# huster-wgm/SRCGAN

Hardware: AMD Instinct MI355X
Metric: paired SR-CycleGAN train images/sec at x4 256->1024 (higher is better)
Workload: dtype bf16; 1 GPU; Sat2Aerx4 paired G+D step (BASELINE configs[1]): 23-block RRDB generator + 3-layer PatchGAN, 3x256x256->3x1024x1024, batch 16/GPU; per_gpu_batch=16, global_batch=16, parallelism=dp1, gradient_exchange=none (1 rank)

## Files before the change

include/srcgan_amd.h:

```cpp
#ifndef SRCGAN_AMD_H
#define SRCGAN_AMD_H

#include <stddef.h>
#include <stdint.h>

#ifdef __cplusplus
extern "C" {
#endif

#define SRCGAN_F32 0
#define SRCGAN_BF16 1
#define SRCGAN_F16 2

int srcgan_version(void);
const char* srcgan_last_error(void);
int srcgan_dtype_size(int dtype);

int srcgan_nchw_f32_to_nhwc(const float* src, void* dst, int B, int C, int H, int W,
                            int cs, int dtype, void* stream);
int srcgan_nhwc_to_nchw_f32(const void* src, float* dst, int B, int C, int H, int W,
                            int cs, int coff, int dtype, void* stream);

size_t srcgan_packed_weight_bytes(int rows, int kdim, int ntaps, int dtype);
int srcgan_pack_weight(const float* w, void* wp, int rows, int kdim, int tys, int txs,
// ... 19 lines not shown
    long x_plane, y_plane, r1_plane, r2_plane, mz_plane;
    int rev_batch;
    void* sign_out; const void* sign_in;
    int npar; long wpar_stride;
} srcgan_conv_desc;
int srcgan_conv_igemm(const srcgan_conv_desc* d, void* stream);

typedef struct srcgan_wgrad_desc {
    const void* dy; const void* x; float* slab; float* grad;
    float* bias_grad;
    int dtype;
    int kh, kw, stride;
    int B, H, W, Cin, x_cs, x_coff;
    int OH, OW, Cout, dy_cs, dy_coff;
    int pad_y, pad_x;
    int nsplit;
    long sr, sk, sty, stx, off;
    float alpha;
    int accumulate;
} srcgan_wgrad_desc;
size_t srcgan_conv_wgrad_slab_bytes(int Cout, int Cin, int kh, int kw, int nsplit);
int srcgan_conv_wgrad_nsplit(int B, int OH, int OW, int Cout, int Cin, int stride);
int srcgan_conv_wgrad(const srcgan_wgrad_desc* d, void* stream);

typedef struct srcgan_wgrad_seg { int g0, g1; float* grad; float* bias; int Cin; float alpha; } srcgan_wgrad_seg;
typedef struct srcgan_wgrad_dense_desc {
    const void* dy; const void* x; float* slab;
    int dtype;
    int B, H, W;
    int G, dy_cs, dy_coff;
    int C, x_cs, x_coff;
    int nseg;
    srcgan_wgrad_seg seg[8];
    int accumulate;
    long dy_plane, x_plane;
} srcgan_wgrad_dense_desc;
size_t srcgan_wgrad_dense_slab_bytes(int G, int C, int dtype, int B, int H, int W);
int srcgan_wgrad_dense(const srcgan_wgrad_dense_desc* d, void* stream);

int srcgan_col_reduce_blocks(long npix);
int srcgan_col_reduce(int mode, const void* a, int a_cs, int a_coff, const void* z, int z_cs, int z_coff,
                      const float* m, const float* rstd, long npix, int C, float scale,
                      float* out0, float* out1, float* scratch, int dtype, void* stream);

int srcgan_bn_finalize(const float* mean, const float* var, float* rstd, float* running_mean,
                       float* running_var, int64_t* num_batches_tracked, int C, long count,
// ... 353 lines not shown
```

srcgan_amd/_native.py:

```python
from __future__ import annotations

import ctypes as C
import os
from typing import Optional, Sequence

import torch

_HERE = os.path.dirname(os.path.abspath(__file__))
LIB_PATH = os.environ.get("SRCGAN_AMD_LIB") or os.path.join(_HERE, "lib", "libsrcgan_amd.so")

F32, BF16, F16 = 0, 1, 2
_DTYPES = {"fp32": F32, "f32": F32, "float32": F32, torch.float32: F32,
           "bf16": BF16, "bfloat16": BF16, torch.bfloat16: BF16,
           "fp16": F16, "f16": F16, "float16": F16, "half": F16, torch.float16: F16, F32: F32, BF16: BF16, F16: F16}
_default_dtype = _DTYPES[os.environ.get("SRCGAN_AMD_DTYPE", "fp32")]


def dtype_id(d) -> int:
    if d is None:
        return _default_dtype
    try:
        return _DTYPES[d]
    except KeyError:
        raise ValueError(f"unsupported compute dtype {d!r} (use 'fp32', 'bf16' or 'fp16')") from None
# ... 27 lines not shown

class WgradDesc(C.Structure):
    _fields_ = [("dy", C.c_void_p), ("x", C.c_void_p), ("slab", C.c_void_p), ("grad", C.c_void_p), ("bias_grad", C.c_void_p),
                ("dtype", C.c_int), ("kh", C.c_int), ("kw", C.c_int), ("stride", C.c_int),
                ("B", C.c_int), ("H", C.c_int), ("W", C.c_int), ("Cin", C.c_int), ("x_cs", C.c_int), ("x_coff", C.c_int),
                ("OH", C.c_int), ("OW", C.c_int), ("Cout", C.c_int), ("dy_cs", C.c_int), ("dy_coff", C.c_int),
                ("pad_y", C.c_int), ("pad_x", C.c_int), ("nsplit", C.c_int),
                ("sr", C.c_long), ("sk", C.c_long), ("sty", C.c_long), ("stx", C.c_long), ("off", C.c_long),
                ("alpha", C.c_float), ("accumulate", C.c_int)]


class WgradSeg(C.Structure):
    _fields_ = [("g0", C.c_int), ("g1", C.c_int), ("grad", C.c_void_p), ("bias", C.c_void_p), ("Cin", C.c_int), ("alpha", C.c_float)]


class WgradDenseDesc(C.Structure):
    _fields_ = [("dy", C.c_void_p), ("x", C.c_void_p), ("slab", C.c_void_p), ("dtype", C.c_int),
                ("B", C.c_int), ("H", C.c_int), ("W", C.c_int),
                ("G", C.c_int), ("dy_cs", C.c_int), ("dy_coff", C.c_int),
                ("C", C.c_int), ("x_cs", C.c_int), ("x_coff", C.c_int),
                ("nseg", C.c_int), ("seg", WgradSeg * 8), ("accumulate", C.c_int), ("dy_plane", C.c_long), ("x_plane", C.c_long)]


class RddbCfg(C.Structure):
    _fields_ = [("in_ch", C.c_int), ("out_ch", C.c_int), ("up", C.c_int), ("nf", C.c_int), ("nb", C.c_int), ("gc", C.c_int),
                ("B", C.c_int), ("H", C.c_int), ("W", C.c_int), ("dtype", C.c_int), ("down", C.c_int), ("legacy", C.c_int)]


class NetOpts(C.Structure):
    _fields_ = [("wpack", C.c_void_p), ("pack", C.c_int), ("rrdb_lo", C.c_int), ("rrdb_hi", C.c_int), ("guard", C.c_void_p)]


class ResDeconvCfg(C.Structure):
    _fields_ = [("in_ch", C.c_int), ("out_ch", C.c_int), ("B", C.c_int), ("H", C.c_int), ("W", C.c_int), ("dtype", C.c_int),
                ("layers", C.c_int * 4), ("norm", C.c_int)]


class SrNetCfg(C.Structure):
    _fields_ = [(n, C.c_int) for n in ("kind", "in_ch", "out_ch", "up", "base", "B", "H", "W", "dtype", "nres")]


class SrDenseCfg(C.Structure):
    _fields_ = [(n, C.c_int) for n in ("kind", "in_ch", "out_ch", "B", "H", "W", "dtype", "growth", "num_blocks", "num_layers", "up")]


class RcanCfg(C.Structure):
# ... 20 lines not shown
class VggLossCfg(C.Structure):
    _fields_ = [(n, C.c_int) for n in ("kind", "B", "H", "W", "dtype")]


class NLayerDCfg(C.Structure):
    _fields_ = [("in_ch", C.c_int), ("ndf", C.c_int), ("n_layers", C.c_int),
                ("B", C.c_int), ("H", C.c_int), ("W", C.c_int), ("dtype", C.c_int), ("training", C.c_int), ("norm", C.c_int)]


_P, _I, _L, _F, _S = C.c_void_p, C.c_int, C.c_long, C.c_float, C.c_size_t
SIGNATURES = {
    "srcgan_version": (_I, []),
    "srcgan_last_error": (C.c_char_p, []),
    "srcgan_dtype_size": (_I, [_I]),
    "srcgan_nchw_f32_to_nhwc": (_I, [_P, _P, _I, _I, _I, _I, _I, _I, _P]),
    "srcgan_nhwc_to_nchw_f32": (_I, [_P, _P, _I, _I, _I, _I, _I, _I, _I, _P]),
    "srcgan_packed_weight_bytes": (_S, [_I, _I, _I, _I]),
    "srcgan_pack_weight": (_I, [_P, _P, _I, _I, _I, _I, _L, _L, _L, _L, _L, _I, _P]),
    "srcgan_pack_weight_part": (_I, [_P, _P, _I, _I, _I, _I, _L, _L, _L, _L, _L, _I, _I, _F, _I, _P]),
    "srcgan_conv_igemm": (_I, [C.POINTER(ConvDesc), _P]),
    "srcgan_conv_wgrad_slab_bytes": (_S, [_I, _I, _I, _I, _I]),
    "srcgan_conv_wgrad_nsplit": (_I, [_I, _I, _I, _I, _I, _I]),
    "srcgan_conv_wgrad": (_I, [C.POINTER(WgradDesc), _P]),
    "srcgan_wgrad_dense_slab_bytes": (_S, [_I, _I, _I, _I, _I, _I]),
    "srcgan_wgrad_dense": (_I, [C.POINTER(WgradDenseDesc), _P]),
    "srcgan_col_reduce_blocks": (_I, [_L]),
    "srcgan_col_reduce": (_I, [_I, _P, _I, _I, _P, _I, _I, _P, _P, _L, _I, _F, _P, _P, _P, _I, _P]),
    "srcgan_bn_finalize": (_I, [_P, _P, _P, _P, _P, _P, _I, _L, _F, _F, _P]),
    "srcgan_bn_eval_rstd": (_I, [_P, _P, _I, _F, _P]),
    "srcgan_bn_apply_lrelu": (_I, [_P, _P, _P, _P, _P, _P, _L, _I, _I, _F, _I, _P]),
    "srcgan_bn_bwd_apply": (_I, [_P, _P, _P, _P, _P, _P, _P, _P, _L, _I, _I, _I, _P]),
    "srcgan_add_inplace": (_I, [_P, _I, _I, _P, _I, _I, _P, _I, _I, _F, _L, _I, _I, _P]),
    "srcgan_add_inplace_planes": (_I, [_P, _I, _I, _L, _P, _I, _I, _L, _P, _I, _I, _L, _F, _L, _I, _I, _P]),
    "srcgan_gn_scratch_floats": (_S, [_I, _I]),
    "srcgan_gn_forward": (_I, [_P, _I, _P, _I, _P, _I, _P, _P, _P, _I, _L, _I, _I, _F, _I, _F, _I, _P, _P]),
    "srcgan_gn_backward": (_I, [_P, _I, _P, _I, _P, _I, _P, _P, _P, _I, _P, _I, _I, _P, _P, _I, _F, _I, _L, _I, _I, _I, _P, _P]),
    "srcgan_ca_scratch_floats": (_S, [_I, _L, _I]),
    "srcgan_ca_forward": (_I, [_P, _I, _P, _I, _P, _I, _P, _P, _P, _P, _P, _I, _L, _I, _I, _I, _P, _P]),
    "srcgan_ca_backward": (_I, [_P, _I, _P, _I, _P, _P, _P, _P, _I, _P, _I, _I, _P, _P, _P, _P, _I, _L, _I, _I, _I, _P, _P]),
    "srcgan_s2d_shift": (_I, [_P, _I, _P, _I, _I, _I, _I, _I, _I, _I, _I, _I, _I, _P]),
    "srcgan_d2s_shift": (_I, [_P, _I, _P, _I, _I, _I, _I, _I, _I, _I, _I, _I, _I, _I, _P]),
    "srcgan_prelu_forward": (_I, [_P, _I, _P, _P, _P, _I, _F, _P, _I, _I, _I, _I, _I, _I, _I, _I, _I, _I, _P]),
    "srcgan_prelu_scratch_floats": (_S, [_I, _I, _I, _I, _I]),
    "srcgan_prelu_backward": (_I, [_P, _I, _P, _I, _P, _P, _P, _I, _P, _I, _F, _I, _P, _P, _I, _I, _I, _I, _I, _I, _I, _I, _I, _P, _P]),
    "srcgan_upsample2_nhwc": (_I, [_P, _I, _I, _L, _P, _I, _I, _I, _I, _I, _I, _P]),
    "srcgan_sum2x2_nhwc": (_I, [_P, _I, _P, _I, _P, _I, _F, _I, _I, _I, _I, _I, _P]),
# ... 191 lines not shown
```

srcgan_amd/build.py:

```python
import glob
import os
import subprocess
import sys
from concurrent.futures import ThreadPoolExecutor

HERE = os.path.dirname(os.path.abspath(__file__))
CSRC = os.path.join(HERE, "csrc")
LIBDIR = os.path.join(HERE, "lib")
LIB = os.path.join(LIBDIR, "libsrcgan_amd.so")
SOURCES = ["conv_entry.hip", "conv_igemm.hip", "conv_par4.hip", "deconv_k3s2.hip", "conv3x3_dma.hip", "conv_wgrad.hip", "wgrad_dense.hip", "elementwise.hip", "class_losses.hip", "groupnorm.hip", "chan_attn.hip", "back_proj.hip", "metrics.hip", "shift_select.hip", "scene_score.hip", "colour.hip", "tiles.hip", "vgg_loss.hip", "nets.hip", "oplist.hip"]
FLAGS = ["--offload-arch=gfx950", "-O3", "-std=c++17", "-fPIC", "-Wall", "-Wno-unused-function"]


def _hipcc():
    for c in (os.environ.get("HIPCC"), "/opt/rocm/bin/hipcc", "hipcc"):
        if c and (os.path.isabs(c) and os.path.exists(c) or not os.path.isabs(c)):
            return c
    raise RuntimeError("hipcc not found")


def _stale(target, deps):
    if not os.path.exists(target):
        return True
    t = os.path.getmtime(target)
    return any(os.path.getmtime(d) > t for d in deps)


def build(force=False, verbose=True):
    os.makedirs(LIBDIR, exist_ok=True)
    hipcc = _hipcc()
    headers = glob.glob(os.path.join(CSRC, "*.h")) + [os.path.join(HERE, "..", "include", "srcgan_amd.h")]
    objs, jobs = [], []
    for s in SOURCES:
# ... 23 lines not shown
```

srcgan_amd/csrc/common.h:

```cpp
#pragma once
#include <hip/hip_runtime.h>
#include <stdint.h>
#include <stdio.h>
#include <stdarg.h>
#include <string.h>
#include "../../include/srcgan_amd.h"

typedef __attribute__((ext_vector_type(8))) __bf16 bf16x8;
typedef __attribute__((ext_vector_type(8))) _Float16 f16x8;
typedef __attribute__((ext_vector_type(4))) _Float16 f16x4;
typedef __attribute__((ext_vector_type(4))) __bf16 bf16x4;
typedef __attribute__((ext_vector_type(4))) float f32x4;
typedef __attribute__((ext_vector_type(16))) float f32x16;
typedef __attribute__((ext_vector_type(4))) short s16x4;
typedef __attribute__((ext_vector_type(4))) unsigned int u32x4;
typedef __attribute__((ext_vector_type(2))) unsigned int u32x2;

template <typename T> struct DT;
template <> struct DT<float>  { static constexpr int id = SRCGAN_F32;  static constexpr int EPP = 4; static constexpr int KCE = 16; };
template <> struct DT<__bf16> { static constexpr int id = SRCGAN_BF16; static constexpr int EPP = 8; static constexpr int KCE = 32; };
template <> struct DT<_Float16> { static constexpr int id = SRCGAN_F16; static constexpr int EPP = 8; static constexpr int KCE = 32; };
static inline bool sg_is16(int dtype) { return dtype == SRCGAN_BF16 || dtype == SRCGAN_F16; }
static inline bool sg_dtype_ok(int dtype) { return dtype == SRCGAN_F32 || sg_is16(dtype); }

// ... 79 lines not shown
#endif
#endif

int sg_prof_start(const char* cls, double flops, double bytes, hipStream_t st);
void sg_prof_stop(int token, hipStream_t st);

struct SgPackJob {
    const float* w; size_t wp_off;
    int rows, kdim, tys, txs;
    long sr, sk, sty, stx, off;
    int k_off, k_total; float scale;
    int cot, nchunk; long total, blk0;
};
void sg_pack_job_finish(SgPackJob& j, int dtype, long& blk_cursor);
int sg_pack_multi_launch(const SgPackJob* jobs_dev, int njobs, long nblocks, void* wp_base, int dtype, hipStream_t st, const unsigned long long* guard = nullptr);
int sg_fold_tail_pack(const float* w_deconv, const float* w_conv, void* wp, int tar, int dtype, hipStream_t st);
void sg_minmax_frames(const float* x, int planes, int frames, long n, int nblk, float* partial, float* range, hipStream_t st);
int sg_vgg_combine(const float* sums, const float* weights, int n, float* out, hipStream_t st);
struct SgFrames { int Cin, F, f0, k; };
int sg_frames_pack(const float* src5d, void* dst, int cs, int Bt, SgFrames fr, int H, int W, int dtype, hipStream_t st);
int sg_frames_grad_store(const void* src, int cs, float* dst5d, int Bt, SgFrames fr, int H, int W, const float* gout, float gscale, int dtype, hipStream_t st);
int sg_meanshift(const void* x, void* y, const float* w, const float* bias, int transpose, long npix, int dtype, hipStream_t st);
int sg_proj_repack(const float* src, float* dst, int form, int rows, int kdim, int k, int s, int back, hipStream_t st);
int sg_fill_zero_guarded(void* p, size_t bytes, const unsigned long long* guard, hipStream_t st);
```

srcgan_amd/csrc/conv_wgrad.hip:

```cpp
#include "launch.h"
#include <type_traits>

struct WgradP {
    const void* dy; const void* x; float* slab;
    int B, H, W, Cin, xCs, xcoff;
    int OH, OW, Cout, dyCs, dycoff;
    int pad_y, pad_x;
    int nsplit, tiles_x, tiles_y, ntiles, citiles, ctiles, want_bias;
};

typedef __attribute__((address_space(3))) s16x4 lds_s16x4;

__device__ __forceinline__ bf16x8 tr_frag(const char* p0, const char* p1) {
    s16x4 lo = __builtin_amdgcn_ds_read_tr16_b64_v4i16((lds_s16x4*)(p0));
    s16x4 hi = __builtin_amdgcn_ds_read_tr16_b64_v4i16((lds_s16x4*)(p1));
    typedef __attribute__((ext_vector_type(8))) short s16x8;
    s16x8 v = {lo[0], lo[1], lo[2], lo[3], hi[0], hi[1], hi[2], hi[3]};
    return __builtin_bit_cast(bf16x8, v);
}

template <typename T, int KH, int KW, int S, int MT, int TH, int NCW, bool BIASW>
__global__ __launch_bounds__((NCW + (BIASW ? 1 : 0)) * 64) void conv_wgrad_k(const WgradP p) {
    using D = DT<T>;
    constexpr int NW = NCW + (BIASW ? 1 : 0);
// ... 323 lines not shown
        s = (a0 + a1) + (a2 + a3);
    }
    red[sl][el] = s;
    __syncthreads();
    if (sl != 0 || e >= per_split) return;
    s = (red[0][el] + red[1][el]) + (red[2][el] + red[3][el]);
    long q = e;
    const int ci_l = (int)(q % 32); q /= 32;
    const int co_l = (int)(q % p.COT); q /= p.COT;
    const int tap = (int)(q % (p.ntap + 1)); q /= (p.ntap + 1);
    const int cit = (int)(q % p.citiles);
    const int ct = (int)(q / p.citiles);
    const int co = ct * p.COT + co_l, ci = cit * 32 + ci_l;
    if (co >= p.Cout) return;
    const float v = s * p.alpha;
    if (tap == p.ntap) {
        if (p.bias_grad && cit == 0 && ci_l == 0) p.bias_grad[co] = p.accumulate ? p.bias_grad[co] + v : v;
        return;
    }
    if (ci >= p.Cin) return;
    const int ky = tap / p.kw, kx = tap % p.kw;
    float* g = p.grad + p.off + co * p.sr + ci * p.sk + ky * p.sty + kx * p.stx;
    *g = p.accumulate ? (*g + v) : v;
}

static inline int wg_cot(int Cout) { return Cout <= 32 ? 32 : 64; }

extern "C" size_t srcgan_conv_wgrad_slab_bytes(int Cout, int Cin, int kh, int kw, int nsplit) {
    const int cot = wg_cot(Cout);
    return (size_t)nsplit * cdiv(Cout, cot) * cdiv(Cin, 32) * (kh * kw + 1) * cot * 32 * sizeof(float);
}

extern "C" int srcgan_conv_wgrad_nsplit(int B, int OH, int OW, int Cout, int Cin, int stride) {
    const int th = stride == 2 ? 4 : 8;
    const long ntiles = (long)B * cdiv(OH, th) * cdiv(OW, 32);
    const long pairs = (long)cdiv(Cout, wg_cot(Cout)) * cdiv(Cin, 32);
    long want = cdivl(1024, pairs);
    if (want > ntiles) want = ntiles;
    if (want > 256) want = 256;
    if (want < 1) want = 1;
    return (int)want;
}

template <typename T, int KH, int KW, int S, int MT, int TH, int NCW, bool BIASW>
static int launch_wgrad(WgradP p, hipStream_t st) {
    constexpr int NW = NCW + (BIASW ? 1 : 0);
// ... 69 lines not shown
    int rc;
    const bool c3 = d->kh == 3 && d->kw == 3 && d->Cout <= 3 && d->OH == d->H && d->OW == d->W;
    const bool c1 = d->kh == 4 && d->kw == 4 && d->Cout == 1 && d->OH == d->H - 1 && d->OW == d->W - 1;
    if (sg_is16(d->dtype) && (c3 || c1) && d->stride == 1 && d->pad_y == 1 && d->pad_x == 1 && !d->bias_grad && d->Cin % 32 == 0) {
        p.tiles_x = cdiv(p.W, 32); p.tiles_y = cdiv(p.H, 8); p.ntiles = p.B * p.tiles_x * p.tiles_y;
        p.nsplit = d->nsplit;
        if (p.nsplit > p.ntiles) p.nsplit = p.ntiles;
        const dim3 grid((unsigned)(p.citiles * ((p.nsplit + 7) / 8) * 8), 1, 1);
        const double px = (double)p.B * p.OH * p.OW;
        rc = sg_dtype_dispatch16(d->dtype, [&](auto t) {
            using T = decltype(t);
            char cls[96];
            snprintf(cls, sizeof(cls), "conv_wgrad<%s,%s>", sg_dtype_tag<T>(), c3 ? "3x3,s1,c3" : "4x4,s1,c1");
            const int tok = sg_prof_start(cls, 2.0 * px * d->kh * d->kw * d->Cin * d->Cout, ((double)p.B * p.H * p.W * d->Cin + px * d->Cout) * 2, st);
            if (c3) hipLaunchKernelGGL((wgrad_c3_k<T, 3, 3>), grid, dim3(256), 0, st, p);
            else hipLaunchKernelGGL((wgrad_c3_k<T, 4, 1>), grid, dim3(256), 0, st, p);
            sg_prof_stop(tok, st);
            SG_LAUNCH_CHECK();
            return 0;
        });
    } else if (cot == 32) rc = sg_dtype_dispatch(d->dtype, [&](auto t) { return dispatch_wgrad<decltype(t), 1>(p, d->kh, d->kw, d->stride, st); });
    else rc = sg_dtype_dispatch(d->dtype, [&](auto t) { return dispatch_wgrad<decltype(t), 2>(p, d->kh, d->kw, d->stride, st); });
    if (rc) return rc;
    WredP q;
    q.slab = d->slab; q.grad = d->grad; q.bias_grad = d->bias_grad; q.nsplit = p.nsplit; q.ctiles = p.ctiles; q.citiles = p.citiles;
    q.ntap = d->kh * d->kw; q.kw = d->kw; q.COT = cot; q.Cout = d->Cout; q.Cin = d->Cin;
    q.sr = d->sr; q.sk = d->sk; q.sty = d->sty; q.stx = d->stx; q.off = d->off;
    q.alpha = d->alpha; q.accumulate = d->accumulate;
    const long per_split = (long)p.ctiles * p.citiles * (q.ntap + 1) * cot * 32;
    hipLaunchKernelGGL(wgrad_reduce_k, dim3((unsigned)cdivl(per_split, 64)), dim3(256), 0, st, q);
    SG_LAUNCH_CHECK();
    return 0;
}
```

srcgan_amd/csrc/nets.hip:

```cpp
#include "net_common.h"
#include <map>
#include <mutex>
#include <string>

int sg_zigzag_next() {
    static const bool zig = sg_env("SRCGAN_NO_ZIGZAG") == nullptr;
    static int flip = 0;
    const int rev = flip;
    flip ^= 1;
    return zig ? rev : 0;
}

namespace {
struct PackCache { std::vector<SgPackJob> host; SgPackJob* dev = nullptr; SgPackJob* pinned = nullptr; size_t cap = 0; hipEvent_t staged = nullptr; };
std::map<std::string, PackCache> g_pack_cache;
std::mutex g_pack_mutex;
}

int sg_pack_list_run(const std::vector<SgPackJob>& jobs, long nblk, void* wp_base, int dtype, const char* tag, const void* key_ptr, void* st,
                     const unsigned long long* guard) {
    if (jobs.empty()) return 0;
    int dev = 0;
    SG_HIP(hipGetDevice(&dev));
    char key[112];
// ... 198 lines not shown
    }
    if (P.nrr) N.home = b.take((size_t)((nf + P.kce - 1) / P.kce) * P.plane_bytes);
    if (P.family != RDDB_LEGACY) N.T = b.take(B * P.Ht * P.Wt * nf * e);
    if (P.x2_tail) {
        N.U[0] = b.take(B * P.Ht * P.Wt * nf * e);
        size_t pp[2];
        for (int k = 0; k < 2; ++k) pp[k] = b.take(B * P.HO * P.WO * nf * e);
        for (int k = 0; k < P.ntail; ++k) N.tail[k] = pp[k & 1];
    } else if (P.family == RDDB_SRDN) {
        N.U[0] = N.T;
    } else {
        size_t pp[2] = {0, 0};
        for (int k = 0; k < 2 && k <= P.nst; ++k) {
            const int top = ((P.nst - k) & ~1) + k;
            pp[k] = b.take(B * (P.Ht << top) * (P.Wt << top) * nf * e);
        }
        for (int s = 0; s <= P.nst; ++s) N.U[s] = pp[s & 1];
    }
    N.out = b.take(B * P.HO * P.WO * P.out_cs * e);
    N.wpk = b.off;
    N.total = N.wpk + P.wpack_bytes;
}

struct RddbBwdPlan {
    size_t dout, dU[6], Pg[3], szP, dfea_dn[5], dxin, slab, colscr, total;
};
static void rddb_bwd_plan(const srcgan_rddbnet_cfg* c, const RddbPlan& P, RddbBwdPlan& Q) {
    const size_t e = P.esz, B = c->B;
    Bump b;
    Q.dout = b.take(B * P.HO * P.WO * P.out_cs * e);
    for (int s = 0; s <= P.nup; ++s) Q.dU[s] = b.take(B * (P.Ht << s) * (P.Wt << s) * c->nf * e);
    if (P.x2_tail) { Q.dU[1] = b.take(B * P.HO * P.WO * c->nf * e); Q.dU[2] = b.take(B * P.HO * P.WO * c->nf * e); }
    Q.szP = align_up((size_t)P.nplane * P.plane_bytes, 256);
    for (int i = 0; i < 3; ++i) Q.Pg[i] = b.take(Q.szP);
    for (int s = 0; s <= P.ndn; ++s) Q.dfea_dn[s] = b.take(B * (c->H >> s) * (c->W >> s) * c->nf * e);
    Q.dxin = b.take(B * c->H * c->W * P.in_cs * e);
    size_t slab = 0;
    auto mx = [&](size_t v) { if (v > slab) slab = v; };
    mx(wgrad_slab(c->B, c->H, c->W, c->nf, P.in_cs, 3, 3, 1));
    for (int k = 0; k < 5; ++k) mx(wgrad_slab(c->B, P.Ht, P.Wt, k < 4 ? c->gc : c->nf, c->nf + k * c->gc, 3, 3, 1));
    mx(wgrad_slab(c->B, P.Ht, P.Wt, c->nf, c->nf, 3, 3, 1));
    for (int s = 0; s < P.nup; ++s) mx(wgrad_slab(c->B, P.Ht << s, P.Wt << s, c->nf, c->nf, 2, 2, 2));
    for (int k = 0; k < P.ntail; ++k) if (P.tail[k].conv) mx(wgrad_slab(c->B, P.tail[k].hout, P.tail[k].wout, c->nf, c->nf, 3, 3, 1));
    for (int s = 0; s < P.ndn; ++s) mx(wgrad_slab(c->B, c->H >> (s + 1), c->W >> (s + 1), c->nf, c->nf, 3, 3, 2));
    mx(wgrad_slab(c->B, P.HO, P.WO, c->out_ch, c->nf, 3, 3, 1));
    mx(srcgan_wgrad_dense_slab_bytes(P.C, P.C, c->dtype, c->B, P.Ht, P.Wt));
    Q.slab = b.take(slab);
    const long maxpix = (long)B * (P.HO > c->H ? P.HO : c->H) * (P.WO > c->W ? P.WO : c->W);
    Q.colscr = b.take((size_t)2 * srcgan_col_reduce_blocks(maxpix) * P.C * sizeof(float));
    Q.total = b.off + 256;
}

}

extern "C" int srcgan_rddbnet_num_params(const srcgan_rddbnet_cfg* c) { RddbPlan P; if (rddb_plan(c, P)) return -1; return P.nparams; }
extern "C" int srcgan_rddbnet_num_rrdb(const srcgan_rddbnet_cfg* c) { RddbPlan P; if (rddb_plan(c, P)) return -1; return P.nrr; }
extern "C" size_t srcgan_rddbnet_wpack_bytes(const srcgan_rddbnet_cfg* c) { RddbPlan P; if (rddb_plan(c, P)) return 0; return P.wpack_bytes; }
extern "C" size_t srcgan_rddbnet_ws_bytes(const srcgan_rddbnet_cfg* c) {
    RddbPlan P; if (rddb_plan(c, P)) return 0;
    RddbNames N; rddb_train_names(c, P, N); return N.total;
}
extern "C" size_t srcgan_rddbnet_infer_ws_bytes(const srcgan_rddbnet_cfg* c) {
    RddbPlan P; if (rddb_plan(c, P)) return 0;
    RddbNames N; rddb_infer_names(c, P, N); return N.total;
}
// ... 207 lines not shown
        }
    }
    for (int s = 0; s < P.ndn; ++s) P.dn_dgrad().pack(packs, params[P.p_dn0 + 2 * s], wp, P.w_dn_d[s]);
    if (pack_dx) packs.add(params[P.p_first_w], wp + P.w_first_d, c->in_ch, nf, 3, 3, lay_dgrad_s1(c->in_ch, 3, 3));
    return packs.run((std::string(P.tag) + (pack_dx ? "_bwd_dx" : "_bwd")).c_str(), params[0], st, pack_guard(opt));
}

int RddbBwd::output_plain() const {
    TRef Ul = T_(N.U[P.nup], nf);
    if (G(P.p_last_w))
        SG_TRY(wgrad_call(dt, dout(), P.HO, P.WO, c->out_ch, Ul, B, P.HO, P.WO, nf, 3, 3, 1, 1, 1, lay_fwd(nf, 3, 3), 1.f, slab, G(P.p_last_w), st));
    {
        Conv cv(dt, 3, 3, 1);
        cv.in(dout(), B, P.HO, P.WO, P.out_cs).w(wp + P.w_last_d).out(S_(Q.dU[P.nup], nf), P.HO, P.WO, nf).pad(1, 1);
        if (P.nup > 0) {
            if (N.um_bytes) { cv.sign_in(w8 + N.um); cv.d.mslope = 0.2f; }
            else cv.mask(Ul, 0);
        }
        SG_TRY(cv.run(st));
    }
    for (int s = P.nup - 1; s >= 0; --s) {
        const int h = H << s, w = W << s;
        TRef dHR = S_(Q.dU[s + 1], nf), Us = T_(N.U[s], nf);
        if (G(P.p_up0 + s))
            SG_TRY(wgrad_call(dt, Us, h, w, nf, dHR, B, 2 * h, 2 * w, nf, 2, 2, 2, 0, 0, WLayout{(long)nf * 4, 4, 2, 1, 0}, 1.f, slab, G(P.p_up0 + s), st));
        Conv cv(dt, 2, 2, 2);
        cv.in(dHR, B, 2 * h, 2 * w, nf).w(wp + P.w_up_d[s]).out(S_(Q.dU[s], nf), h, w, nf).pad(0, 0);
        if (s > 0) cv.mask(Us, 0);
        SG_TRY(cv.run(st));
    }
    return 0;
}

int RddbBwd::output_tail() const {
    TRef tin = P.family == RDDB_LEGACY ? Abuf(0) : T_(N.U[0], nf);
    auto obuf = [&](int k) { return k < 0 ? tin : T_(N.tail[k], nf); };
    TRef Fl = obuf(P.ntail - 1);
    if (G(P.p_last_w))
        SG_TRY(wgrad_call(dt, dout(), P.HO, P.WO, c->out_ch, Fl, B, P.HO, P.WO, nf, 3, 3, 1, 1, 1, lay_fwd(nf, 3, 3), 1.f, slab, G(P.p_last_w), st, G(P.p_last_b)));
    else if (G(P.p_last_b)) SG_TRY(bias_grad(dt, dout(), (long)B * P.HO * P.WO, c->out_ch, 1.f, G(P.p_last_b), colscr, st));
    int pp = 0;
    auto nextbuf = [&](int k_in) { if (k_in < 0) return dU0(); pp ^= 1; return S_(Q.dU[1 + pp], nf); };
    TRef dcur = nextbuf(P.ntail - 1);
    {
        Conv cv(dt, 3, 3, 1);
        cv.in(dout(), B, P.HO, P.WO, P.out_cs).w(wp + P.w_last_d).out(dcur, P.HO, P.WO, nf).pad(1, 1);
// ... 447 lines not shown
```

srcgan_amd/ops.py:

```python
from __future__ import annotations

import ctypes as C
from typing import Optional, Tuple

import torch

from . import _native as N

TORCH_DT = {N.F32: torch.float32, N.BF16: torch.bfloat16, N.F16: torch.float16}


def to_nhwc(x: torch.Tensor, cs: Optional[int] = None, dtype=None) -> torch.Tensor:
    N.require_cuda(x, "to_nhwc")
    dt = N.dtype_id(dtype)
    x = x.contiguous().float()
    B, Cc, H, W = x.shape
    cs = cs or Cc
    out = torch.empty(B, H, W, cs, dtype=TORCH_DT[dt], device=x.device)
    N.check(N.lib().srcgan_nchw_f32_to_nhwc(x.data_ptr(), out.data_ptr(), B, Cc, H, W, cs, dt, N.stream_ptr(x.device)), "to_nhwc")
    return out


def to_nchw(x: torch.Tensor, Cc: Optional[int] = None, coff: int = 0) -> torch.Tensor:
    N.require_cuda(x, "to_nchw")
# ... 118 lines not shown
               dy_coff: int = 0, x_coff: int = 0, pad: Tuple[int, int] = (0, 0), layout: Tuple[int, int, int, int, int],
               alpha: float = 1.0, nsplit: Optional[int] = None, accumulate: bool = False,
               bias_grad: Optional[torch.Tensor] = None) -> torch.Tensor:
    N.require_cuda(x, "conv_wgrad")
    lib = N.lib()
    d = N.WgradDesc()
    B, OH, OW, dycs = dy.shape
    _, H, W, xcs = x.shape
    ns = nsplit or lib.srcgan_conv_wgrad_nsplit(B, OH, OW, Cout, Cin, stride)
    slab = torch.empty(lib.srcgan_conv_wgrad_slab_bytes(Cout, Cin, kh, kw, ns), dtype=torch.uint8, device=x.device)
    d.dy, d.x, d.slab, d.grad = dy.data_ptr(), x.data_ptr(), slab.data_ptr(), grad.data_ptr()
    d.bias_grad = bias_grad.data_ptr() if bias_grad is not None else None
    d.dtype = N.dtype_id(x.dtype)
    d.kh, d.kw, d.stride = kh, kw, stride
    d.B, d.H, d.W, d.Cin, d.x_cs, d.x_coff = B, H, W, Cin, xcs, x_coff
    d.OH, d.OW, d.Cout, d.dy_cs, d.dy_coff = OH, OW, Cout, dycs, dy_coff
    d.pad_y, d.pad_x, d.nsplit = pad[0], pad[1], ns
    d.sr, d.sk, d.sty, d.stx, d.off = layout
    d.alpha, d.accumulate = alpha, int(accumulate)
    N.check(lib.srcgan_conv_wgrad(C.byref(d), N.stream_ptr(x.device)), "srcgan_conv_wgrad")
    return grad


def wgrad_dense(dy: torch.Tensor, x: torch.Tensor, segs, *, G: Optional[int] = None, Cc: Optional[int] = None,
                dy_plane: int = 0, x_plane: int = 0, shape: Optional[Tuple[int, int, int]] = None) -> None:
    N.require_cuda(x, "wgrad_dense")
    lib = N.lib()
    d = N.WgradDenseDesc()
    if shape is not None:
        (B, H, W), dycs = shape, dy.shape[-1]
    else:
        B, H, W, dycs = dy.shape
    G = G or dycs
    Cc = Cc or x.shape[-1]
    dt = N.dtype_id(x.dtype)
    slab = torch.empty(lib.srcgan_wgrad_dense_slab_bytes(G, Cc, dt, B, H, W), dtype=torch.uint8, device=x.device)
    d.dy, d.x, d.slab, d.dtype = dy.data_ptr(), x.data_ptr(), slab.data_ptr(), dt
    d.B, d.H, d.W, d.G, d.dy_cs, d.dy_coff, d.C, d.x_cs, d.x_coff = B, H, W, G, dycs, 0, Cc, x.shape[-1], 0
    d.dy_plane, d.x_plane = dy_plane, x_plane
    d.nseg = len(segs)
    for i, (g0, g1, grad, bias, cin, alpha) in enumerate(segs):
        d.seg[i].g0, d.seg[i].g1, d.seg[i].Cin, d.seg[i].alpha = g0, g1, cin, alpha
        d.seg[i].grad = grad.data_ptr() if grad is not None else None
        d.seg[i].bias = bias.data_ptr() if bias is not None else None
    N.check(lib.srcgan_wgrad_dense(C.byref(d), N.stream_ptr(x.device)), "srcgan_wgrad_dense")

# ... 115 lines not shown
```

Before: 122.2 images/s.

## Fuse k2s2 upsample deconv weight-grad and input-grad into one pass

```diff
diff --git a/include/srcgan_amd.h b/include/srcgan_amd.h
--- a/include/srcgan_amd.h
+++ b/include/srcgan_amd.h
@@ -65,6 +65,20 @@
 size_t srcgan_conv_wgrad_slab_bytes(int Cout, int Cin, int kh, int kw, int nsplit);
 int srcgan_conv_wgrad_nsplit(int B, int OH, int OW, int Cout, int Cin, int stride);
 int srcgan_conv_wgrad(const srcgan_wgrad_desc* d, void* stream);
+
+typedef struct srcgan_deconv_k2s2_bwd_desc {
+    const void* dhr; const void* u; const void* wp; void* du;
+    float* slab; float* grad;
+    int dtype;
+    int B, H, W;
+    int mask; float mslope;
+    int accumulate;
+    int nwg;
+} srcgan_deconv_k2s2_bwd_desc;
+int srcgan_deconv_k2s2_bwd_ok(int dtype, int nf, int W);
+int srcgan_deconv_k2s2_bwd_nwg(int B, int H, int W, int ncu);
+size_t srcgan_deconv_k2s2_bwd_slab_bytes(int nwg);
+int srcgan_deconv_k2s2_bwd(const srcgan_deconv_k2s2_bwd_desc* d, void* stream);
 
 typedef struct srcgan_wgrad_seg { int g0, g1; float* grad; float* bias; int Cin; float alpha; } srcgan_wgrad_seg;
 typedef struct srcgan_wgrad_dense_desc {
diff --git a/srcgan_amd/_native.py b/srcgan_amd/_native.py
--- a/srcgan_amd/_native.py
+++ b/srcgan_amd/_native.py
@@ -73,6 +73,12 @@
                 ("nseg", C.c_int), ("seg", WgradSeg * 8), ("accumulate", C.c_int), ("dy_plane", C.c_long), ("x_plane", C.c_long)]
 
 
+class DeconvK2S2BwdDesc(C.Structure):
+    _fields_ = [("dhr", C.c_void_p), ("u", C.c_void_p), ("wp", C.c_void_p), ("du", C.c_void_p), ("slab", C.c_void_p), ("grad", C.c_void_p),
+                ("dtype", C.c_int), ("B", C.c_int), ("H", C.c_int), ("W", C.c_int), ("mask", C.c_int), ("mslope", C.c_float),
+                ("accumulate", C.c_int), ("nwg", C.c_int)]
+
+
 class RddbCfg(C.Structure):
     _fields_ = [("in_ch", C.c_int), ("out_ch", C.c_int), ("up", C.c_int), ("nf", C.c_int), ("nb", C.c_int), ("gc", C.c_int),
                 ("B", C.c_int), ("H", C.c_int), ("W", C.c_int), ("dtype", C.c_int), ("down", C.c_int), ("legacy", C.c_int)]
@@ -139,6 +145,10 @@
     "srcgan_conv_wgrad_slab_bytes": (_S, [_I, _I, _I, _I, _I]),
     "srcgan_conv_wgrad_nsplit": (_I, [_I, _I, _I, _I, _I, _I]),
     "srcgan_conv_wgrad": (_I, [C.POINTER(WgradDesc), _P]),
+    "srcgan_deconv_k2s2_bwd_ok": (_I, [_I, _I, _I]),
+    "srcgan_deconv_k2s2_bwd_nwg": (_I, [_I, _I, _I, _I]),
+    "srcgan_deconv_k2s2_bwd_slab_bytes": (_S, [_I]),
+    "srcgan_deconv_k2s2_bwd": (_I, [C.POINTER(DeconvK2S2BwdDesc), _P]),
     "srcgan_wgrad_dense_slab_bytes": (_S, [_I, _I, _I, _I, _I, _I]),
     "srcgan_wgrad_dense": (_I, [C.POINTER(WgradDenseDesc), _P]),
     "srcgan_col_reduce_blocks": (_I, [_L]),
diff --git a/srcgan_amd/build.py b/srcgan_amd/build.py
--- a/srcgan_amd/build.py
+++ b/srcgan_amd/build.py
@@ -8,7 +8,7 @@
 CSRC = os.path.join(HERE, "csrc")
 LIBDIR = os.path.join(HERE, "lib")
 LIB = os.path.join(LIBDIR, "libsrcgan_amd.so")
-SOURCES = ["conv_entry.hip", "conv_igemm.hip", "conv_par4.hip", "deconv_k3s2.hip", "conv3x3_dma.hip", "conv_wgrad.hip", "wgrad_dense.hip", "elementwise.hip", "class_losses.hip", "groupnorm.hip", "chan_attn.hip", "back_proj.hip", "metrics.hip", "shift_select.hip", "scene_score.hip", "colour.hip", "tiles.hip", "vgg_loss.hip", "nets.hip", "oplist.hip"]
+SOURCES = ["conv_entry.hip", "conv_igemm.hip", "conv_par4.hip", "deconv_k3s2.hip", "deconv_k2s2_bwd.hip","conv3x3_dma.hip", "conv_wgrad.hip", "wgrad_dense.hip", "elementwise.hip", "class_losses.hip", "groupnorm.hip", "chan_attn.hip", "back_proj.hip", "metrics.hip", "shift_select.hip", "scene_score.hip", "colour.hip", "tiles.hip", "vgg_loss.hip", "nets.hip", "oplist.hip"]
 FLAGS = ["--offload-arch=gfx950", "-O3", "-std=c++17", "-fPIC", "-Wall", "-Wno-unused-function"]
 
 
diff --git a/srcgan_amd/csrc/common.h b/srcgan_amd/csrc/common.h
--- a/srcgan_amd/csrc/common.h
+++ b/srcgan_amd/csrc/common.h
@@ -125,4 +125,6 @@
 int sg_frames_grad_store(const void* src, int cs, float* dst5d, int Bt, SgFrames fr, int H, int W, const float* gout, float gscale, int dtype, hipStream_t st);
 int sg_meanshift(const void* x, void* y, const float* w, const float* bias, int transpose, long npix, int dtype, hipStream_t st);
 int sg_proj_repack(const float* src, float* dst, int form, int rows, int kdim, int k, int s, int back, hipStream_t st);
+int sg_wgrad_reduce(const float* slab, float* grad, float* bias_grad, int nsplit, int ctiles, int citiles, int ntap, int kw, int cot, int Cout, int Cin,
+                    long sr, long sk, long sty, long stx, long off, float alpha, int accumulate, hipStream_t st);
 int sg_fill_zero_guarded(void* p, size_t bytes, const unsigned long long* guard, hipStream_t st);
diff --git a/srcgan_amd/csrc/conv_wgrad.hip b/srcgan_amd/csrc/conv_wgrad.hip
--- a/srcgan_amd/csrc/conv_wgrad.hip
+++ b/srcgan_amd/csrc/conv_wgrad.hip
@@ -369,6 +369,19 @@
     const int ky = tap / p.kw, kx = tap % p.kw;
     float* g = p.grad + p.off + co * p.sr + ci * p.sk + ky * p.sty + kx * p.stx;
     *g = p.accumulate ? (*g + v) : v;
+}
+
+int sg_wgrad_reduce(const float* slab, float* grad, float* bias_grad, int nsplit, int ctiles, int citiles, int ntap, int kw, int cot, int Cout, int Cin,
+                    long sr, long sk, long sty, long stx, long off, float alpha, int accumulate, hipStream_t st) {
+    WredP q;
+    q.slab = slab; q.grad = grad; q.bias_grad = bias_grad; q.nsplit = nsplit; q.ctiles = ctiles; q.citiles = citiles;
+    q.ntap = ntap; q.kw = kw; q.COT = cot; q.Cout = Cout; q.Cin = Cin;
+    q.sr = sr; q.sk = sk; q.sty = sty; q.stx = stx; q.off = off;
+    q.alpha = alpha; q.accumulate = accumulate;
+    const long per_split = (long)ctiles * citiles * (ntap + 1) * cot * 32;
+    hipLaunchKernelGGL(wgrad_reduce_k, dim3((unsigned)cdivl(per_split, 64)), dim3(256), 0, st, q);
+    SG_LAUNCH_CHECK();
+    return 0;
 }
 
 static inline int wg_cot(int Cout) { return Cout <= 32 ? 32 : 64; }
@@ -484,13 +497,6 @@
     } else if (cot == 32) rc = sg_dtype_dispatch(d->dtype, [&](auto t) { return dispatch_wgrad<decltype(t), 1>(p, d->kh, d->kw, d->stride, st); });
     else rc = sg_dtype_dispatch(d->dtype, [&](auto t) { return dispatch_wgrad<decltype(t), 2>(p, d->kh, d->kw, d->stride, st); });
     if (rc) return rc;
-    WredP q;
-    q.slab = d->slab; q.grad = d->grad; q.bias_grad = d->bias_grad; q.nsplit = p.nsplit; q.ctiles = p.ctiles; q.citiles = p.citiles;
-    q.ntap = d->kh * d->kw; q.kw = d->kw; q.COT = cot; q.Cout = d->Cout; q.Cin = d->Cin;
-    q.sr = d->sr; q.sk = d->sk; q.sty = d->sty; q.stx = d->stx; q.off = d->off;
-    q.alpha = d->alpha; q.accumulate = d->accumulate;
-    const long per_split = (long)p.ctiles * p.citiles * (q.ntap + 1) * cot * 32;
-    hipLaunchKernelGGL(wgrad_reduce_k, dim3((unsigned)cdivl(per_split, 64)), dim3(256), 0, st, q);
-    SG_LAUNCH_CHECK();
-    return 0;
-}
+    return sg_wgrad_reduce(d->slab, d->grad, d->bias_grad, p.nsplit, p.ctiles, p.citiles, d->kh * d->kw, d->kw, cot, d->Cout, d->Cin,
+                           d->sr, d->sk, d->sty, d->stx, d->off, d->alpha, d->accumulate, st);
+}
diff --git a/srcgan_amd/csrc/deconv_k2s2_bwd.hip b/srcgan_amd/csrc/deconv_k2s2_bwd.hip
--- /dev/null
+++ b/srcgan_amd/csrc/deconv_k2s2_bwd.hip
@@ -0,0 +1,198 @@
+#include "launch.h"
+
+struct UpBwdP {
+    const char* dhr; const char* u; const char* wp; char* du; float* slab;
+    int W, rows;
+    int tiles_x, ntiles, nwg;
+    int mask; float mslope;
+};
+
+typedef __attribute__((address_space(3))) void* ub_lptr_t;
+constexpr int UB_OOB = 0x7fffffff;
+typedef int ub_v4i __attribute__((ext_vector_type(4)));
+__device__ __forceinline__ void ub_dma16(const void* base, int voff, int soff, ub_lptr_t lds) {
+    const unsigned long long a = (unsigned long long)base;
+    ub_v4i rs;
+    rs[0] = __builtin_amdgcn_readfirstlane((int)(a & 0xffffffffu));
+    rs[1] = __builtin_amdgcn_readfirstlane((int)((a >> 32) & 0xffffu));
+    rs[2] = 0x7fffffff;
+    rs[3] = 0x00020000;
+    const unsigned dst = __builtin_amdgcn_readfirstlane((unsigned)(unsigned long long)lds);
+    unsigned keep;
+    asm volatile("s_mov_b32 %0, m0\n\ts_mov_b32 m0, %3\n\ts_nop 0\n\tbuffer_load_dwordx4 %1, %2, %4 offen lds\n\ts_mov_b32 m0, %0"
+                 : "=&s"(keep) : "v"(voff), "s"(rs), "s"(dst), "s"(soff) : "memory");
+}
+typedef __attribute__((address_space(3))) s16x4 ub_lds_s16x4;
+typedef __attribute__((address_space(3))) bf16x8 ub_lds_bf16x8;
+
+__device__ __forceinline__ bf16x8 ub_tr_frag(unsigned a0, unsigned a1) {
+    s16x4 lo = __builtin_amdgcn_ds_read_tr16_b64_v4i16((ub_lds_s16x4*)(uintptr_t)a0);
+    s16x4 hi = __builtin_amdgcn_ds_read_tr16_b64_v4i16((ub_lds_s16x4*)(uintptr_t)a1);
+    typedef __attribute__((ext_vector_type(8))) short s16x8;
+    s16x8 v = {lo[0], lo[1], lo[2], lo[3], hi[0], hi[1], hi[2], hi[3]};
+    return __builtin_bit_cast(bf16x8, v);
+}
+__device__ __forceinline__ bf16x8 ub_ld16(unsigned a) { return *(const ub_lds_bf16x8*)(uintptr_t)a; }
+
+constexpr int UB_DBYTES = 2 * 256 * 64, UB_UBYTES = 2 * 64 * 64, UB_SBYTES = UB_DBYTES + UB_UBYTES;
+constexpr size_t UB_SMEM = 2 * (size_t)UB_SBYTES;
+static_assert(UB_SMEM <= 80 * 1024, "two workgroups per CU");
+
+template <typename T>
+__global__ __launch_bounds__(512) __attribute__((amdgpu_waves_per_eu(4, 4))) void deconv_k2s2_bwd_k(const UpBwdP p) {
+    typedef __attribute__((ext_vector_type(8))) T vecT;
+    extern __shared__ __attribute__((aligned(1024))) char smem[];
+    const int tid = threadIdx.x, lane = tid & 63;
+    const int wave = __builtin_amdgcn_readfirstlane(tid >> 6);
+    int v = blockIdx.x;
+    if ((p.nwg & 7) == 0) v = (v & 7) * (p.nwg >> 3) + (v >> 3);
+    const int t_begin = (int)((long)p.ntiles * v / p.nwg), t_end = (int)((long)p.ntiles * (v + 1) / p.nwg);
+
+    const unsigned loff = (unsigned)((lane >> 2) * 128 + (lane & 3) * 16);
+    const int u_row = (wave & 3) >> 1;
+    const int u_uni = (u_row * p.W + (wave & 1) * 16) * 128 + (wave >> 2) * 64;
+    const int d_uni = ((wave >> 2) * 2 * p.W + (wave & 3) * 16) * 128, d_row2 = 2 * 2 * p.W * 128;
+    auto issue = [&](int rp, int tx, int stage) {
+        const bool row1 = 2 * rp + 1 < p.rows;
+        const char* dorg = p.dhr + ((size_t)(4 * rp) * (2 * p.W) + 64 * tx) * 128;
+        const char* uorg = p.u + ((size_t)(2 * rp) * p.W + 32 * tx) * 128;
+        char* ls = smem + stage * UB_SBYTES;
+#pragma unroll
+        for (int it = 0; it < 4; ++it)
+            ub_dma16(dorg, (row1 || (it & 1) == 0) ? (int)loff : UB_OOB, d_uni + (it & 1) * d_row2 + (it >> 1) * 64, (ub_lptr_t)(ls + (it * 8 + wave) * 1024));
+        ub_dma16(uorg, (row1 || u_row == 0) ? (int)loff : UB_OOB, u_uni, (ub_lptr_t)(ls + (32 + wave) * 1024));
+    };
+
+    const int r = lane & 31, h = lane >> 5;
+    const int gq = lane >> 4, idx = lane & 15, qq = idx >> 2, pp = idx & 3;
+    const int choff = ((gq & 1) * 16 + 4 * pp) * 2;
+    const int wtap = wave & 3, wa = wtap >> 1, wb = wtap & 1, wn = wave >> 2;
+    const unsigned wa_lane = (unsigned)((8 * h + qq) * 64 + choff);
+    const unsigned wb_lane = 2 * wa_lane - (unsigned)choff;
+    const unsigned wb_uni = (unsigned)(wn * 16384 + (wa * 64 + wb) * 64);
+    f32x16 wacc[2];
+#pragma unroll
+    for (int m = 0; m < 2; ++m)
+#pragma unroll
+        for (int i = 0; i < 16; ++i) wacc[m][i] = 0.f;
+
+    const int chalf = wave & 1, grp = wave >> 1, gpy = grp >> 1, gxb = (grp & 1) * 16, q4 = lane >> 4;
+    const unsigned dg_lane = (unsigned)((lane & 15) * 64 + q4 * 16);
+    const unsigned dg_uni = (unsigned)((2 * gpy * 64 + 2 * gxb) * 64), mk_uni = (unsigned)(UB_DBYTES + chalf * 4096 + (gpy * 32 + gxb) * 64);
+    const int st_lane = (lane & 15) * 128 + q4 * 16, st_uni = (gpy * p.W + gxb) * 128 + chalf * 64;
+    bf16x8 wreg[2][8];
+#pragma unroll
+    for (int blk = 0; blk < 2; ++blk) {
+        const int rho = lane & 15, ci = chalf * 32 + 8 * (rho >> 2) + 4 * blk + (rho & 3);
+#pragma unroll
+        for (int ks = 0; ks < 8; ++ks)
+            wreg[blk][ks] = *(const bf16x8*)(p.wp + (((ks & 1) * 4 + (ks >> 1)) * 64 + ci) * 64 + q4 * 16);
+    }
+
+    const unsigned lds0 = (unsigned)(unsigned long long)(ub_lptr_t)smem;
+    int rp = t_begin / p.tiles_x, tx = t_begin - rp * p.tiles_x;
+    if (t_begin < t_end) issue(rp, tx, 0);
+    int stage = 0;
+    for (int t = t_begin; t < t_end; ++t, stage ^= 1) {
+        int rpn = rp, txn = tx + 1;
+        if (txn == p.tiles_x) { txn = 0; ++rpn; }
+        __builtin_amdgcn_s_waitcnt(0x0f70);
+        __syncthreads();
+        if (t + 1 < t_end) issue(rpn, txn, stage ^ 1);
+        const unsigned ld = lds0 + stage * UB_SBYTES;
+        {
+            const unsigned ab = ld + UB_DBYTES + wa_lane, bb = ld + wb_uni + wb_lane;
+#pragma unroll
+            for (int kk = 0; kk < 4; ++kk) {
+                const int py = kk >> 1, xh = (kk & 1) * 16;
+                const unsigned bo = (unsigned)((2 * py * 64 + 2 * xh) * 64), ao = (unsigned)((py * 32 + xh) * 64);
+                const bf16x8 bv = ub_tr_frag(bb + bo, bb + bo + 8 * 64);
+#pragma unroll
+                for (int m = 0; m < 2; ++m)
+                    wacc[m] = sg_mfma16<T>(ub_tr_frag(ab + ao + m * 4096, ab + ao + m * 4096 + 4 * 64), bv, wacc[m]);
+            }
+        }
+        f32x4 d0 = {0.f, 0.f, 0.f, 0.f}, d1 = {0.f, 0.f, 0.f, 0.f};
+        {
+            const unsigned gb = ld + dg_uni + 2 * dg_lane - (unsigned)(q4 * 16);
+#pragma unroll
+            for (int ks = 0; ks < 8; ++ks) {
+                const int tap = ks >> 1, a = tap >> 1, b = tap & 1;
+                const bf16x8 bf = ub_ld16(gb + (unsigned)((ks & 1) * 16384 + (a * 64 + b) * 64));
+                d0 = sg_mfma16s<T>(wreg[0][ks], bf, d0);
+                d1 = sg_mfma16s<T>(wreg[1][ks], bf, d1);
+            }
+        }
+        float o[8] = {d0[0], d0[1], d0[2], d0[3], d1[0], d1[1], d1[2], d1[3]};
+        if (p.mask) {
+            const vecT z = __builtin_bit_cast(vecT, ub_ld16(ld + mk_uni + dg_lane));
+#pragma unroll
+            for (int i = 0; i < 8; ++i) o[i] *= to_f(z[i]) > 0.f ? 1.f : p.mslope;
+        }
+        vecT ov;
+#pragma unroll
+        for (int i = 0; i < 8; ++i) ov[i] = from_f<T>(o[i]);
+        const __amdgpu_buffer_rsrc_t dd = __builtin_amdgcn_make_buffer_rsrc(p.du + ((size_t)(2 * rp) * p.W + 32 * tx) * 128, 0, 0x7fffffff, 0x00020000u);
+        __builtin_amdgcn_raw_buffer_store_b128(__builtin_bit_cast(u32x4, ov), dd, 2 * rp + gpy < p.rows ? st_lane : UB_OOB, st_uni, 0);
+        rp = rpn; tx = txn;
+    }
+
+    float* sp = p.slab + (((size_t)v * 2 + wn) * 5 + wtap) * (64 * 32);
+#pragma unroll
+    for (int m = 0; m < 2; ++m)
+#pragma unroll
+        for (int i = 0; i < 16; ++i) sp[(m * 32 + 8 * (i >> 2) + 4 * h + (i & 3)) * 32 + r] = wacc[m][i];
+}
+
+extern "C" int srcgan_deconv_k2s2_bwd_ok(int dtype, int nf, int W) { return sg_is16(dtype) && nf == 64 && W > 0 && W % 32 == 0; }
+
+static long ub_ntiles(int B, int H, int W) { return cdivl((long)B * H, 2) * (W / 32); }
+
+extern "C" int srcgan_deconv_k2s2_bwd_nwg(int B, int H, int W, int ncu) {
+    const long ntiles = ub_ntiles(B, H, W);
+    long n = 2L * (ncu > 0 ? ncu : 256);
+    if (n > ntiles) n = ntiles;
+    if (n >= 8) n -= n % 8;
+    return (int)(n < 1 ? 1 : n);
+}
+
+extern "C" size_t srcgan_deconv_k2s2_bwd_slab_bytes(int nwg) { return (size_t)nwg * 2 * 5 * 64 * 32 * sizeof(float); }
+
+extern "C" int srcgan_deconv_k2s2_bwd(const srcgan_deconv_k2s2_bwd_desc* d, void* stream) {
+    SG_REQUIRE(d && d->dhr && d->u && d->wp && d->du && d->slab && d->grad, "srcgan_deconv_k2s2_bwd: null pointer");
+    SG_REQUIRE(sg_is16(d->dtype), "srcgan_deconv_k2s2_bwd: 16-bit modes only (dtype %d)", d->dtype);
+    SG_REQUIRE(d->B > 0 && d->H > 0 && d->W > 0 && d->W % 32 == 0, "srcgan_deconv_k2s2_bwd: W must be a positive multiple of 32 (B=%d H=%d W=%d)", d->B, d->H, d->W);
+    SG_REQUIRE((long)d->W * 8 * 128 < (1L << 31) && (long)d->B * d->H < (1L << 29), "srcgan_deconv_k2s2_bwd: a tile's extent must fit 31 bits");
+    SG_REQUIRE(((uintptr_t)d->dhr % 16) == 0 && ((uintptr_t)d->u % 16) == 0 && ((uintptr_t)d->du % 16) == 0 && ((uintptr_t)d->wp % 16) == 0,
+               "srcgan_deconv_k2s2_bwd: tensors must be 16-byte aligned");
+    hipStream_t st = (hipStream_t)stream;
+    int dev = 0;
+    SG_TRY(sg_current_device(dev));
+    UpBwdP p;
+    memset(&p, 0, sizeof(p));
+    p.dhr = (const char*)d->dhr; p.u = (const char*)d->u; p.wp = (const char*)d->wp; p.du = (char*)d->du; p.slab = d->slab;
+    p.W = d->W; p.rows = d->B * d->H; p.tiles_x = d->W / 32; p.ntiles = (int)ub_ntiles(d->B, d->H, d->W);
+    p.mask = d->mask; p.mslope = d->mslope;
+    if (d->nwg > 0) p.nwg = d->nwg;
+    else {
+        const int ncu = sg_cu_count(dev);
+        if (ncu <= 0) return 1;
+        p.nwg = srcgan_deconv_k2s2_bwd_nwg(d->B, d->H, d->W, ncu);
+    }
+    SG_REQUIRE(p.nwg <= p.ntiles, "srcgan_deconv_k2s2_bwd: %d workgroups for %d tiles", p.nwg, p.ntiles);
+    const double px = (double)d->B * d->H * d->W;
+    int rc = sg_dtype_dispatch16(d->dtype, [&](auto t) {
+        using T = decltype(t);
+        constexpr auto kern = deconv_k2s2_bwd_k<T>;
+        SG_TRY(sg_allow_lds<kern>(UB_SMEM, dev));
+        char cls[96];
+        snprintf(cls, sizeof(cls), "deconv_k2s2_bwd<%s>", sg_dtype_tag<T>());
+        const int tok = sg_prof_start(cls, 2.0 * 2.0 * px * 256 * 64, px * (4 * 128 + 128 + 128), st);
+        hipLaunchKernelGGL(kern, dim3((unsigned)p.nwg), dim3(512), UB_SMEM, st, p);
+        sg_prof_stop(tok, st);
+        SG_LAUNCH_CHECK();
+        return 0;
+    });
+    if (rc) return rc;
+    return sg_wgrad_reduce(d->slab, d->grad, nullptr, p.nwg, 1, 2, 4, 2, 64, 64, 64, 64L * 4, 4, 2, 1, 0, 1.f, d->accumulate, st);
+}
diff --git a/srcgan_amd/csrc/nets.hip b/srcgan_amd/csrc/nets.hip
--- a/srcgan_amd/csrc/nets.hip
+++ b/srcgan_amd/csrc/nets.hip
@@ -244,6 +244,12 @@
     N.total = N.wpk + P.wpack_bytes;
 }
 
+static bool up_bwd_fused(int dtype, int nf, int w) {
+    static const bool split = sg_env("SRCGAN_UPBWD_SPLIT") != nullptr;
+    return !split && srcgan_deconv_k2s2_bwd_ok(dtype, nf, w);
+}
+static int up_bwd_nwg(int B, int h, int w) { return srcgan_deconv_k2s2_bwd_nwg(B, h, w, 256); }
+
 struct RddbBwdPlan {
     size_t dout, dU[6], Pg[3], szP, dfea_dn[5], dxin, slab, colscr, total;
 };
@@ -262,7 +268,10 @@
     mx(wgrad_slab(c->B, c->H, c->W, c->nf, P.in_cs, 3, 3, 1));
     for (int k = 0; k < 5; ++k) mx(wgrad_slab(c->B, P.Ht, P.Wt, k < 4 ? c->gc : c->nf, c->nf + k * c->gc, 3, 3, 1));
     mx(wgrad_slab(c->B, P.Ht, P.Wt, c->nf, c->nf, 3, 3, 1));
-    for (int s = 0; s < P.nup; ++s) mx(wgrad_slab(c->B, P.Ht << s, P.Wt << s, c->nf, c->nf, 2, 2, 2));
+    for (int s = 0; s < P.nup; ++s) {
+        mx(wgrad_slab(c->B, P.Ht << s, P.Wt << s, c->nf, c->nf, 2, 2, 2));
+        if (srcgan_deconv_k2s2_bwd_ok(c->dtype, c->nf, P.Wt << s)) mx(srcgan_deconv_k2s2_bwd_slab_bytes(up_bwd_nwg(c->B, P.Ht << s, P.Wt << s)));
+    }
     for (int k = 0; k < P.ntail; ++k) if (P.tail[k].conv) mx(wgrad_slab(c->B, P.tail[k].hout, P.tail[k].wout, c->nf, c->nf, 3, 3, 1));
     for (int s = 0; s < P.ndn; ++s) mx(wgrad_slab(c->B, c->H >> (s + 1), c->W >> (s + 1), c->nf, c->nf, 3, 3, 2));
     mx(wgrad_slab(c->B, P.HO, P.WO, c->out_ch, c->nf, 3, 3, 1));
@@ -516,6 +525,14 @@
     for (int s = P.nup - 1; s >= 0; --s) {
         const int h = H << s, w = W << s;
         TRef dHR = S_(Q.dU[s + 1], nf), Us = T_(N.U[s], nf);
+        if (G(P.p_up0 + s) && up_bwd_fused(dt, nf, w)) {
+            srcgan_deconv_k2s2_bwd_desc d;
+            memset(&d, 0, sizeof(d));
+            d.dhr = dHR.p; d.u = Us.p; d.wp = wp + P.w_up_d[s]; d.du = s8 + Q.dU[s]; d.slab = slab; d.grad = G(P.p_up0 + s);
+            d.dtype = dt; d.B = B; d.H = h; d.W = w; d.mask = s > 0; d.mslope = 0.2f; d.nwg = up_bwd_nwg(B, h, w);
+            SG_TRY(srcgan_deconv_k2s2_bwd(&d, st));
+            continue;
+        }
         if (G(P.p_up0 + s))
             SG_TRY(wgrad_call(dt, Us, h, w, nf, dHR, B, 2 * h, 2 * w, nf, 2, 2, 2, 0, 0, WLayout{(long)nf * 4, 4, 2, 1, 0}, 1.f, slab, G(P.p_up0 + s), st));
         Conv cv(dt, 2, 2, 2);
diff --git a/srcgan_amd/ops.py b/srcgan_amd/ops.py
--- a/srcgan_amd/ops.py
+++ b/srcgan_amd/ops.py
@@ -164,6 +164,26 @@
     return grad
 
 
+def deconv_k2s2_bwd(dhr: torch.Tensor, u: torch.Tensor, w: torch.Tensor, grad: torch.Tensor, *, mask: bool = False, mslope: float = 0.2,
+                    accumulate: bool = False, nwg: int = 0, packed: Optional[torch.Tensor] = None,
+                    du: Optional[torch.Tensor] = None) -> torch.Tensor:
+    N.require_cuda(u, "deconv_k2s2_bwd")
+    lib = N.lib()
+    B, H, W, _ = u.shape
+    dt = N.dtype_id(u.dtype)
+    wp = packed if packed is not None else pack_weight(w.float(), 64, 64, 2, 2, 256, 4, 2, 1, 0, u.dtype)
+    if du is None:
+        du = torch.empty_like(u)
+    n = nwg or lib.srcgan_deconv_k2s2_bwd_nwg(B, H, W, torch.cuda.get_device_properties(u.device).multi_processor_count)
+    slab = torch.empty(lib.srcgan_deconv_k2s2_bwd_slab_bytes(n), dtype=torch.uint8, device=u.device)
+    d = N.DeconvK2S2BwdDesc()
+    d.dhr, d.u, d.wp, d.du, d.slab, d.grad = dhr.data_ptr(), u.data_ptr(), wp.data_ptr(), du.data_ptr(), slab.data_ptr(), grad.data_ptr()
+    d.dtype, d.B, d.H, d.W = dt, B, H, W
+    d.mask, d.mslope, d.accumulate, d.nwg = int(mask), mslope, int(accumulate), n
+    N.check(lib.srcgan_deconv_k2s2_bwd(C.byref(d), N.stream_ptr(u.device)), "srcgan_deconv_k2s2_bwd")
+    return du
+
+
 def wgrad_dense(dy: torch.Tensor, x: torch.Tensor, segs, *, G: Optional[int] = None, Cc: Optional[int] = None,
                 dy_plane: int = 0, x_plane: int = 0, shape: Optional[Tuple[int, int, int]] = None) -> None:
     N.require_cuda(x, "wgrad_dense")
```

Measured after the change: 122.7 images/s (median of 6 runs). Within noise of the previous version (+0.5%).
